# nanoporetech/vbz_compression

Measured on AMD Instinct MI355X. Metric: MB/s encode+decode, int16 signal, 1/2/4/8 MI355X vs CPU; ratio preserved, higher is better.
Workload: dtype int16

## Files before the change

### vbz_compression_amd/csrc/zstd_encode.hip

```cpp
#include "vbz_kernels.h"
#include "zstd_entropy.h"

namespace vbzhip {

namespace {

constexpr int WAVE = 64;
constexpr uint32_t BLOCK_MAX = 128u << 10;
constexpr uint32_t MIN_BLOCK = 4096;
constexpr uint32_t HUF_BLOCK_MAX = 92u << 10;
constexpr uint32_t SPLIT_MIN = 2048;
constexpr int MAXBLK = 16;
#ifndef VBZ_SPAN_BLOCK_KB
#define VBZ_SPAN_BLOCK_KB 16
#endif
constexpr uint32_t SPAN_BLOCK = VBZ_SPAN_BLOCK_KB << 10;
#ifndef VBZ_SPAN_SMALL_BLOCKS
#define VBZ_SPAN_SMALL_BLOCKS 2
#endif
constexpr uint32_t SPAN_BYTES_SMALL = SPAN_BLOCK * VBZ_SPAN_SMALL_BLOCKS, SPAN_BYTES_LARGE = SPAN_BLOCK * MAXBLK;
constexpr uint32_t SPAN_LARGE_FROM = 256u << 20;
#ifndef VBZ_KEYSPAN_KB
#define VBZ_KEYSPAN_KB 8
#endif
constexpr uint32_t KEYSPAN_BYTES = VBZ_KEYSPAN_KB << 10, KEYSPAN_LARGE_FROM = 1u << 20;
#ifndef VBZ_KEYSPAN_SHARED_KB
#define VBZ_KEYSPAN_SHARED_KB 4
#endif
constexpr uint32_t KEYSPAN_BYTES_SHARED = VBZ_KEYSPAN_SHARED_KB << 10;
__host__ __device__ constexpr uint32_t keyspan_bytes_for(uint32_t K) { return K >= KEYSPAN_LARGE_FROM ? 2u * KEYSPAN_BYTES : KEYSPAN_BYTES; }
__host__ __device__ constexpr uint32_t span_bytes_for(uint32_t N) { return N >= SPAN_LARGE_FROM ? SPAN_BYTES_LARGE : SPAN_BYTES_SMALL; }
#ifndef VBZ_STEP_LANE
#define VBZ_STEP_LANE 16
#endif
constexpr int STEP_LANE = VBZ_STEP_LANE;
static_assert(STEP_LANE == 16, "the packing step is written for 16 symbols per lane");
constexpr int STEP_DW = STEP_LANE / 4;
constexpr int STEP_SYMS = WAVE * STEP_LANE;
constexpr int OBUF_WORDS = (STEP_SYMS * 11) / 32 + 8;

struct EncSpan
{
    uint32_t read;
    uint32_t r0, r1;
    uint32_t flags;
    uint64_t tmp_off;
    uint32_t tmp_cap;
    uint32_t ord;
};
constexpr uint32_t SPAN_FIRST = 1, SPAN_LAST = 2, SPAN_KEYSEQ = 4, SPAN_SKIP = 8;
constexpr uint32_t SPAN_SHARED = 16;
constexpr uint32_t SPAN_TREE = 32;

constexpr uint32_t SHSPAN_BYTES = 8u << 10, SHSPAN_BATCH_FROM = 20u << 20;
constexpr uint32_t SHSPAN_BYTES_LARGE = 4u * SPAN_BLOCK;
constexpr uint32_t SHSPAN_MIN_REGION = 2u * SHSPAN_BYTES;

struct SpanRegion
{
    uint32_t hist[256];
    uint32_t done;
    uint32_t nshared;
    uint32_t mode;
    uint32_t treeSize, huffLog;
    uint32_t pad0[3];
    uint32_t ctable[256];
    uint32_t tree[34];
    uint32_t pad1[2];
};
constexpr uint32_t SPANREGION_ZEROED = 264;
static_assert(sizeof(SpanRegion) % 16 == 0 && offsetof(SpanRegion, ctable) == 4 * SPANREGION_ZEROED, "SpanRegion");

struct EncLds
{
    uint32_t hist[256];
    uint2 ctable[256];
    uint8_t nbBits[256];
    uint8_t weights[260];
    uint8_t tree[136];
    int32_t treeSize;
    uint32_t mode;
    uint32_t huffLog;
    uint32_t rankcnt[16];
    union
    {
        HufPmWksp pm;
        FseWeightWksp fw;
        struct
        {
            uint32_t ssize[WAVE];
            uint32_t sbeg[WAVE];
            uint32_t scnt[WAVE];
            uint32_t obuf[OBUF_WORDS];
            uint16_t seqcode[8 + 256];
            uint32_t seqpiece[256];
        };
    };
    SeqCTables seq;
    uint32_t cp[64];
    uint32_t cpCount, cpSpacing;
    __device__ __forceinline__ void set_code(uint32_t s, uint32_t code, uint32_t nb) { ctable[s] = make_uint2(code, nb); }
};

struct TableLds
{
    uint32_t hist[256];
    uint32_t ctable[256];
    uint8_t nbBits[256];
    uint8_t weights[260];
    uint8_t tree[136];
    int32_t treeSize;
    uint32_t mode;
    uint32_t huffLog;
    uint32_t rankcnt[16];
    union
    {
        HufPmWksp pm;
        FseWeightWksp fw;
    };
    __device__ __forceinline__ void set_code(uint32_t s, uint32_t code, uint32_t nb) { ctable[s] = code | (nb << 16); }
};
struct TokSeqLds
{
    uint32_t obuf[128];
    uint16_t seqcode[8 + 256];
    uint32_t seqpiece[256];
    SeqCTables seq;
    uint32_t cp[64];
    uint32_t cpCount, cpSpacing;
};

__device__ __forceinline__ void put_le(uint8_t* p, uint64_t v, int n)
{
    for (int i = 0; i < n; ++i) {
        uint32_t byte = (uint32_t)(v >> (8 * i)) & 0xFFu;
        asm volatile("" : "+v"(byte));
        p[i] = (uint8_t)byte;
    }
}

__device__ __forceinline__ uint32_t wave_sum_u32(uint32_t v)
{
    return (uint32_t)__builtin_amdgcn_readlane((int)wave_incl_scan_u32(v), 63);
}

__device__ __forceinline__ uint32_t wave_max_u32(uint32_t v)
{
#define VBZ_DPP_MAX(ctrl, rowmask) do { const uint32_t o_ = (uint32_t)__builtin_amdgcn_update_dpp(0, (int)v, ctrl, rowmask, 0xF, false); v = o_ > v ? o_ : v; } while (0)
    VBZ_DPP_MAX(0x111, 0xF);
    VBZ_DPP_MAX(0x112, 0xF);
    VBZ_DPP_MAX(0x114, 0xF);
    VBZ_DPP_MAX(0x118, 0xF);
    VBZ_DPP_MAX(0x142, 0xA);
    VBZ_DPP_MAX(0x143, 0xC);
#undef VBZ_DPP_MAX
    return (uint32_t)__builtin_amdgcn_readlane((int)v, 63);
}

constexpr uint32_t HIST_SAMPLE_FROM = 32u << 10, HIST_SAMPLE_SEEN = 240;

__device__ __forceinline__ uint32_t hist_sample_bytes(const uint8_t* in, uint32_t n)
{
    const uint32_t head = (uint32_t)((16u - ((uintptr_t)in & 15u)) & 15u);
    const uint32_t h = head < n ? head : n;
    const uint32_t nvec = (n - h) >> 4, tail0 = h + (nvec << 4);
    const uint32_t stripes = (nvec + WAVE - 1) / WAVE, groups = stripes >> 2, last = stripes & 3u;
    uint32_t chunks = groups * WAVE;
    if (last) chunks += (nvec - groups * 4u * WAVE) < (uint32_t)WAVE ? (nvec - groups * 4u * WAVE) : (uint32_t)WAVE;
    return h + (n - tail0) + 16u * chunks;
}

template <class LDS>
__device__ __forceinline__ uint32_t region_histogram(LDS& L, const uint8_t* in, uint32_t n, int lane, bool allow_sample);

template <class LDS>
__device__ __forceinline__ uint32_t region_histogram_from_plan(LDS& L, const uint8_t* in, uint32_t n, int lane, bool allow_sample, const uint32_t* sample, const uint32_t* rest)
{
    uint32_t seen = 0;
    uint32_t c[4];
#pragma unroll
    for (int j = 0; j < 4; ++j) {
        c[j] = sample[lane + 64 * j];
        seen += c[j] ? 1u : 0u;
    }
    seen = wave_sum_u32(seen);
    if (allow_sample && n >= HIST_SAMPLE_FROM && seen >= HIST_SAMPLE_SEEN) {
#pragma unroll
        for (int j = 0; j < 4; ++j) L.hist[lane + 64 * j] = c[j] ? c[j] : 1u;
        wave_lds_sync();
        return hist_sample_bytes(in, n) + (256u - seen);
    }
    if (!rest) return region_histogram(L, in, n, lane, allow_sample);
#pragma unroll
    for (int j = 0; j < 4; ++j) L.hist[lane + 64 * j] = c[j] + rest[lane + 64 * j];
    wave_lds_sync();
    return n;
}

template <class LDS>
__device__ __forceinline__ uint32_t region_histogram(LDS& L, const uint8_t* in, uint32_t n, int lane, bool allow_sample)
{
    static_assert(sizeof(HufPmWksp) >= 4 * 256 * sizeof(uint32_t), "the sub-histograms live in the table-construction workspace");
    uint32_t* sub = reinterpret_cast<uint32_t*>(&L.pm);
    for (int i = lane; i < 4 * 256; i += WAVE) sub[i] = 0;
    wave_lds_sync();
    uint32_t* mine = sub + 256 * (lane & 3);
    const uint32_t head = (uint32_t)((16u - ((uintptr_t)in & 15u)) & 15u);
    const uint32_t h = head < n ? head : n;
    if ((uint32_t)lane < h) atomicAdd(&mine[in[lane]], 1u);
    const uint32_t nvec = (n - h) >> 4;
    const uint4* vp = reinterpret_cast<const uint4*>(in + h);
    const uint32_t tail0 = h + (nvec << 4);
    if (tail0 + (uint32_t)lane < n) atomicAdd(&mine[in[tail0 + lane]], 1u);
    auto count = [&](uint32_t first_stripe, uint32_t stripe_step, uint32_t trip_stripes, int loads) {
        for (uint32_t s0 = first_stripe; s0 * WAVE < nvec; s0 += trip_stripes) {
            uint4 q[4];
#pragma unroll
            for (int u = 0; u < 4; ++u) {
                const uint32_t c = (s0 + (uint32_t)u * stripe_step) * WAVE + (uint32_t)lane;
                q[u] = (u < loads && c < nvec) ? vp[c] : make_uint4(0u, 0u, 0u, 0u);
            }
#pragma unroll
            for (int u = 0; u < 4; ++u) {
                const uint32_t c = (s0 + (uint32_t)u * stripe_step) * WAVE + (uint32_t)lane;
                if (u < loads && c < nvec) {
                    const uint32_t w[4] = { q[u].x, q[u].y, q[u].z, q[u].w };
#pragma unroll
                    for (int k = 0; k < 4; ++k) {
#pragma unroll
                        for (int j = 0; j < 4; ++j) atomicAdd(&mine[(w[k] >> (8 * j)) & 0xFFu], 1u);
                    }
                }
            }
        }
    };
    auto total = [&]() -> uint32_t {
        wave_lds_sync();
        uint32_t seen = 0;
        for (int i = lane; i < 256; i += WAVE) {
            const uint32_t c = sub[i] + sub[256 + i] + sub[512 + i] + sub[768 + i];
            L.hist[i] = c;
            seen += c ? 1u : 0u;
        }
        seen = wave_sum_u32(seen);
        wave_lds_sync();
        return seen;
    };
    if (allow_sample && n >= HIST_SAMPLE_FROM) {
        count(0, 4, 16, 4);
        const uint32_t seen = total();
        if (seen >= HIST_SAMPLE_SEEN) {
            for (int i = lane; i < 256; i += WAVE)
                if (L.hist[i] == 0) L.hist[i] = 1;
            wave_lds_sync();
            return hist_sample_bytes(in, n) + (256u - seen);
        }
        count(1, 1, 4, 3);
    } else {
        count(0, 1, 4, 4);
    }
    (void)total();
    return n;
}

#define SUB(k) do { if (tsub) { unsigned long long tn = __builtin_readcyclecounter(); tsub[k] += tn - *tl; *tl = tn; } } while (0)
template <bool STRICT>
__device__ __forceinline__ uint32_t sorted_count(const uint32_t* arr, uint32_t v, uint32_t top)
{
    uint32_t lo = 0;
    for (uint32_t step = top; step; step >>= 1) {
        const uint32_t x = arr[lo + step - 1];
        lo += (STRICT ? x < v : x <= v) ? step : 0u;
    }
    return lo;
}

template <class LDS>
__device__ __forceinline__ uint32_t huf_build_wave(LDS& L, uint32_t maxSym, uint32_t maxNbBits, int lane, unsigned long long* tsub = nullptr, unsigned long long* tl = nullptr)
{
    HufPmWksp& K = L.pm;
    uint32_t key[4];
    {
        const uint4 h = *reinterpret_cast<const uint4*>(&L.hist[4 * lane]);
        const uint32_t c[4] = { h.x, h.y, h.z, h.w };
#pragma unroll
        for (int j = 0; j < 4; ++j) {
            const uint32_t sy = 4u * (uint32_t)lane + (uint32_t)j;
            key[j] = (sy <= maxSym && c[j]) ? ((c[j] << 8) | (255u - sy)) : 0xFFFFFFFFu;
        }
    }
    for (int i = lane; i < (HUF_MAX_BITS + 1) * 16; i += WAVE) (&K.isPkg[0][0])[i] = 0;
#pragma unroll
    for (int k = 2; k <= 256; k <<= 1) {
#pragma unroll
        for (int d = k >> 1; d > 0; d >>= 1) {
            if (d >= 4) {
                const int m = d >> 2;
                const bool up = ((4 * lane) & k) == 0, lower = (lane & m) == 0;
                const bool keep_min = lower == up;
#pragma unroll
                for (int j = 0; j < 4; ++j) {
                    const uint32_t o = (uint32_t)__shfl_xor((int)key[j], m, 64);
                    const uint32_t mn = o < key[j] ? o : key[j], mx = o < key[j] ? key[j] : o;
                    key[j] = keep_min ? mn : mx;
                }
            } else {
#pragma unroll
                for (int a = 0; a < 4; ++a) {
                    const int bb = a ^ d;
                    if (bb > a) {
                        const bool up = ((4 * lane + a) & k) == 0;
                        const uint32_t mn = key[a] < key[bb] ? key[a] : key[bb], mx = key[a] < key[bb] ? key[bb] : key[a];
                        key[a] = up ? mn : mx;
                        key[bb] = up ? mx : mn;
                    }
                }
            }
        }
    }
    uint32_t n = 0;
    {
        uint32_t w4 = 0;
        uint4 lf;
        uint32_t* lfp = &lf.x;
#pragma unroll
        for (int j = 0; j < 4; ++j) {
            const bool present = key[j] != 0xFFFFFFFFu;
            n += (uint32_t)__popcll(__ballot(present));
            lfp[j] = present ? key[j] >> 8 : 0xFFFFFFFFu;
            w4 |= (255u - (key[j] & 255u)) << (8 * j);
        }
        *reinterpret_cast<uint4*>(&K.leaf[4 * lane]) = lf;
        *reinterpret_cast<uint32_t*>(&K.sym[4 * lane]) = w4;
    }
    wave_lds_sync();
    SUB(6);
    const uint32_t X0 = 2u * n - 2u;
    const uint32_t nj = (n + 63u) >> 6;
    constexpr uint32_t PM_INF = 0xFFFFFFFFu;
    uint32_t ln[4] = { 0, 0, 0, 0 };
    uint32_t lk[8];
    {
        uint4 a = make_uint4(PM_INF, PM_INF, PM_INF, PM_INF), c = a;
        if (lane < 32) {
            a = *reinterpret_cast<const uint4*>(&K.leaf[8 * lane]);
            c = *reinterpret_cast<const uint4*>(&K.leaf[8 * lane + 4]);
        }
        const uint32_t w8[8] = { a.x, a.y, a.z, a.w, c.x, c.y, c.z, c.w };
#pragma unroll
        for (int r = 0; r < 8; ++r) lk[r] = w8[r] == PM_INF ? PM_INF : w8[r] << 1;
    }
    uint32_t m = n >> 1;
    uint32_t pk4[4];
#pragma unroll
    for (int q = 0; q < 4; ++q) {
        const uint32_t t = 4u * (uint32_t)lane + (uint32_t)q;
        pk4[q] = t < m ? ((((lk[2 * q] >> 1) + (lk[2 * q + 1] >> 1)) << 1) | 1u) : PM_INF;
    }
    wave_lds_sync();
    uint64_t* const masks = reinterpret_cast<uint64_t*>(K.merged);
    uint32_t levSame = maxNbBits;
    for (uint32_t lev = 2; lev <= maxNbBits; ++lev) {
        const bool last = lev == maxNbBits;
        uint32_t it[8];
        {
            const int src = 2 * (63 - lane);
#pragma unroll
            for (int r = 0; r < 8; ++r) {
                const uint32_t p = (uint32_t)__shfl((int)pk4[(7 - r) & 3], (src + ((7 - r) >> 2)) & 63, 64);
                it[r] = lane < 32 ? lk[r] : p;
            }
        }
#pragma unroll
        for (int dl = 32; dl >= 1; dl >>= 1) {
            const bool lower = (lane & dl) == 0;
#pragma unroll
            for (int r = 0; r < 8; ++r) {
                const uint32_t o = (uint32_t)__shfl_xor((int)it[r], dl, 64);
                const uint32_t mn = o < it[r] ? o : it[r], mx = o < it[r] ? it[r] : o;
                it[r] = lower ? mn : mx;
            }
        }
#pragma unroll
        for (int d = 4; d >= 1; d >>= 1) {
#pragma unroll
            for (int r = 0; r < 8; ++r) {
                if ((r & d) == 0) {
                    const uint32_t x = it[r], y = it[r | d];
                    it[r] = x < y ? x : y;
                    it[r | d] = x < y ? y : x;
                }
            }
        }
#pragma unroll
        for (int r = 0; r < 8; ++r) {
            const uint64_t bm = __ballot((it[r] & 1u) != 0 && it[r] != PM_INF);
            if (lane == 0) masks[8 * lev + (uint32_t)r] = bm;
        }
        if (last) break;
        const uint32_t size = n + m < X0 ? n + m : X0;
        m = size >> 1;
        bool same = true;
#pragma unroll
        for (int q = 0; q < 4; ++q) {
            const uint32_t t = 4u * (uint32_t)lane + (uint32_t)q;
            const uint32_t v = t < m ? ((((it[2 * q] >> 1) + (it[2 * q + 1] >> 1)) << 1) | 1u) : PM_INF;
            same = same && v == pk4[q];
            pk4[q] = v;
        }
        if (__ballot(!same) == 0) {
            levSame = lev;
            break;
        }
    }
    wave_lds_sync();
    SUB(7);
    {
        uint32_t X = X0;
        for (uint32_t lev = maxNbBits; lev >= 2 && X; --lev) {
            const uint64_t* mk = masks + 8u * (lev < levSame ? lev : levSame);
            uint32_t pk = 0;
#pragma unroll
            for (uint32_t r = 0; r < 8; ++r) {
                const uint32_t cnt = X > r ? (X - r + 7u) >> 3 : 0u;
                const uint64_t lm = cnt >= 64u ? ~0ull : ((1ull << cnt) - 1ull);
                pk += (uint32_t)__popcll(mk[r] & lm);
            }
            const uint32_t nl = X - pk;
#pragma unroll
            for (int j = 0; j < 4; ++j) ln[j] += ((uint32_t)lane + 64u * j) < nl ? 1u : 0u;
            X = 2u * pk;
        }
#pragma unroll
        for (int j = 0; j < 4; ++j) ln[j] += ((uint32_t)lane + 64u * j) < X ? 1u : 0u;
    }
    SUB(8);
    for (int i = lane; i < 256; i += WAVE) L.nbBits[i] = 0;
    if (lane < 16) L.rankcnt[lane] = 0;
    wave_lds_sync();
    maxNbBits = (uint32_t)__builtin_amdgcn_readfirstlane((int)ln[0]);
#pragma unroll
    for (int j = 0; j < 4; ++j) {
        const uint32_t e = (uint32_t)lane + 64u * j;
        if ((uint32_t)j < nj && e < n) {
            L.nbBits[K.sym[e]] = (uint8_t)ln[j];
            atomicAdd(&L.rankcnt[ln[j]], 1u);
        }
    }
    SUB(9);
    wave_lds_sync();
    uint32_t val[HUF_ABS_MAX_BITS + 1];
    {
        uint32_t minv = 0;
#pragma unroll
        for (int n = HUF_ABS_MAX_BITS; n > 0; --n) {
            const uint32_t cnt = (uint32_t)n <= maxNbBits ? L.rankcnt[n] : 0u;
            val[n] = minv;
            minv = (uint32_t)n <= maxNbBits ? ((minv + cnt) >> 1) : 0u;
        }
        val[0] = 0;
    }
    const uint64_t below = (1ull << lane) - 1ull;
#pragma unroll
    for (int j = 0; j < 4; ++j) {
        const uint32_t s = (uint32_t)lane + 64u * j;
        const uint32_t nb = L.nbBits[s];
        uint32_t code = 0;
#pragma unroll
        for (int l = 1; l <= HUF_ABS_MAX_BITS; ++l) {
            const uint64_t m = __ballot(nb == (uint32_t)l);
            if (nb == (uint32_t)l) code = val[l] + (uint32_t)__popcll(m & below);
            val[l] += (uint32_t)__popcll(m);
        }
        L.set_code(s, code, nb);
    }
    wave_lds_sync();
    return maxNbBits;
}

template <class LDS>
__device__ __forceinline__ int huf_write_tree_wave(LDS& L, uint32_t maxSym, uint32_t huffLog, int lane)
{
    FseWeightWksp& W = L.fw;
    const uint32_t wtSize = maxSym;
    const uint32_t cnt = lane <= HUF_ABS_MAX_BITS ? W.count[lane] : 0u;
    const uint64_t nz = __ballot(cnt != 0);
    const uint32_t maxCount = wave_max_u32(cnt);
    bool fast = wtSize > 1 && nz != 0 && maxCount != wtSize && maxCount != 1;
    uint32_t tableLog = 0, maxSV = 0;
    int32_t nm = 0;
    if (fast) {
        maxSV = 63u - (uint32_t)__builtin_clzll(nz);
        tableLog = optimal_table_log(6, wtSize, maxSV, 2);
        const uint32_t total = wtSize;
        const uint64_t scale = 62 - tableLog, step = (1ull << 62) / total, vStep = 1ull << (scale - 20);
        const uint32_t lowThreshold = total >> tableLog;
        int32_t pm = 0;
        if ((uint32_t)lane <= maxSV && cnt) {
            if (cnt <= lowThreshold) nm = 1;
            else {
                int32_t proba = (int32_t)(int16_t)(((uint64_t)cnt * step) >> scale);
                if (proba < 8) {
                    uint32_t rtb = 830000u;
                    rtb = proba == 0 ? 0u : proba == 1 ? 473195u : proba == 2 ? 504333u : proba == 3 ? 520860u
                        : proba == 4 ? 550000u : proba == 5 ? 700000u : proba == 6 ? 750000u : rtb;
                    const uint64_t restToBeat = vStep * rtb;
                    proba += (((uint64_t)cnt * step) - ((uint64_t)proba << scale)) > restToBeat ? 1 : 0;
                }
                nm = proba;
                pm = proba;
            }
        }
        const int32_t still = (int32_t)(1u << tableLog) - (int32_t)wave_sum_u32((uint32_t)nm);
        const uint32_t maxP = wave_max_u32((uint32_t)pm);
        const uint64_t atMax = __ballot(pm > 0 && (uint32_t)pm == maxP);
        const int largest = atMax ? (int)__builtin_ctzll(atMax) : 0;
        const int32_t normLargest = __shfl(nm, largest, 64);
        if (-still >= (normLargest >> 1)) fast = false;
        else if (lane == largest) nm += still;
    }
    if (fast) {
        if (lane < 16) W.norm[lane] = (int16_t)nm;
        for (int i = lane; i < 52; i += WAVE) W.bitbuf[i] = 0;
        wave_lds_sync();
        if (lane == 0) W.verdict = fse_write_ncount(L.tree + 1, 133, W.norm, maxSV, tableLog);
        const uint32_t tableSize = 1u << tableLog, tableMask = tableSize - 1u;
        const uint32_t cum = wave_incl_scan_u32((uint32_t)nm) - (uint32_t)nm;
        if (lane < 16) W.cumul[lane] = cum;
        wave_lds_sync();
        const int hsz = W.verdict;
        if (hsz < 0) fast = false;
        else {
            if ((uint32_t)lane < tableSize) {
                uint32_t sy = 0;
                for (uint32_t u = 1; u <= maxSV; ++u) sy += W.cumul[u] <= (uint32_t)lane ? 1u : 0u;
                W.tableSymbol[((uint32_t)lane * ((tableSize >> 1) + (tableSize >> 3) + 3u)) & tableMask] = (uint8_t)sy;
            }
            if ((uint32_t)lane <= maxSV) {
                uint32_t dnb, dfs = 0;
                if (nm == 0) dnb = ((tableLog + 1) << 16) - tableSize;
                else if (nm == 1) { dnb = (tableLog << 16) - tableSize; dfs = cum - 1u; }
                else {
                    const uint32_t maxBitsOut = tableLog - (uint32_t)hb32((uint32_t)nm - 1u);
                    dnb = (maxBitsOut << 16) - ((uint32_t)nm << maxBitsOut);
                    dfs = cum - (uint32_t)nm;
                }
                W.deltaNbBits[lane] = dnb;
                W.deltaFindState[lane] = (int32_t)dfs;
            }
            wave_lds_sync();
            {
                const bool cell = (uint32_t)lane < tableSize;
                const uint32_t sy = cell ? W.tableSymbol[lane] : 0xFFu;
                uint32_t rank = 0;
                const uint64_t below = (1ull << lane) - 1ull;
                for (uint32_t u = 0; u <= maxSV; ++u) {
                    const uint64_t same = __ballot(sy == u);
                    if (sy == u) rank = (uint32_t)__popcll(same & below);
                }
                if (cell) W.stateTable[W.cumul[sy] + rank] = (uint16_t)(tableSize + (uint32_t)lane);
            }
            wave_lds_sync();
            const uint32_t ne = wtSize - 2u;
            if (lane < 2) {
                const uint32_t s0 = L.weights[wtSize - 1u - (uint32_t)lane];
                const uint32_t d0 = W.deltaNbBits[s0], nb0 = (d0 + (1u << 15)) >> 16;
                uint32_t st = W.stateTable[(int32_t)(((nb0 << 16) - d0) >> nb0) + W.deltaFindState[s0]];
                for (uint32_t k = (uint32_t)lane; k < ne; k += 2) {
                    const uint32_t sy = L.weights[wtSize - 3u - k];
                    const uint32_t nbo = (st + W.deltaNbBits[sy]) >> 16;
                    W.emit[k] = (uint16_t)((st & ((1u << nbo) - 1u)) | (nbo << 8));
                    st = W.stateTable[(int32_t)(st >> nbo) + W.deltaFindState[sy]];
                }
                const uint32_t slot = ne + (((wtSize & 1u) != 0) == (lane == 1) ? 0u : 1u);
                W.emit[slot] = (uint16_t)((st & tableMask) | (tableLog << 8));
                if (lane == 0) W.emit[ne + 2u] = (uint16_t)(1u | (1u << 8));
            }
            wave_lds_sync();
            uint32_t acc = 0, tb = 0;
#pragma unroll
            for (int q = 0; q < 4; ++q) {
                const uint32_t k = 4u * (uint32_t)lane + (uint32_t)q;
                const uint32_t e = k < ne + 3u ? W.emit[k] : 0u;
                acc |= (e & 0xFFu) << tb;
                tb += e >> 8;
            }
            const uint32_t incl = wave_incl_scan_u32(tb);
            const uint32_t off = incl - tb, sh = off & 31u;
            if (tb) {
                atomicOr(&W.bitbuf[off >> 5], acc << sh);
                if (sh + tb > 32u) atomicOr(&W.bitbuf[(off >> 5) + 1u], acc >> (32u - sh));
            }
            const uint32_t nbytes = ((uint32_t)__builtin_amdgcn_readlane((int)incl, 63) + 7u) >> 3;
            wave_lds_sync();
// ... 2232 lines not shown
```

Before: 609,100.

## Add one-symbol-per-lane Huffman builder fast path for alphabets up to 64 symbols

```diff
diff --git a/vbz_compression_amd/csrc/zstd_encode.hip b/vbz_compression_amd/csrc/zstd_encode.hip
--- a/vbz_compression_amd/csrc/zstd_encode.hip
+++ b/vbz_compression_amd/csrc/zstd_encode.hip
@@ -275,6 +275,151 @@
     return lo;
 }
 
+template <int M>
+__device__ __forceinline__ uint32_t lane_xor_u32(uint32_t v)
+{
+    if constexpr (M == 1) return (uint32_t)__builtin_amdgcn_mov_dpp((int)v, 0xB1, 0xF, 0xF, false);
+    else if constexpr (M == 2) return (uint32_t)__builtin_amdgcn_mov_dpp((int)v, 0x4E, 0xF, 0xF, false);
+    else if constexpr (M < 32) return (uint32_t)__builtin_amdgcn_ds_swizzle((int)v, 0x1F | (M << 10));
+    else return (uint32_t)__shfl_xor((int)v, M, 64);
+}
+
+template <class LDS>
+__device__ __forceinline__ uint32_t huf_build_wave_small(LDS& L, uint32_t maxSym, uint32_t maxNbBits, uint32_t n, const uint32_t (&c)[4], int lane,
+                                                         unsigned long long* tsub, unsigned long long* tl)
+{
+    HufPmWksp& K = L.pm;
+    constexpr uint32_t PM_INF = 0xFFFFFFFFu;
+    {
+        uint32_t np = 0;
+#pragma unroll
+        for (int j = 0; j < 4; ++j) np += (4u * (uint32_t)lane + (uint32_t)j <= maxSym && c[j]) ? 1u : 0u;
+        uint32_t pos = wave_incl_scan_u32(np) - np;
+#pragma unroll
+        for (int j = 0; j < 4; ++j) {
+            const uint32_t sy = 4u * (uint32_t)lane + (uint32_t)j;
+            if (sy <= maxSym && c[j]) K.leaf[pos++] = (c[j] << 8) | (255u - sy);
+        }
+    }
+    wave_lds_sync();
+    uint32_t key = (uint32_t)lane < n ? K.leaf[lane] : PM_INF;
+#define VBZ_SORT_STAGE(k, d) do { const uint32_t o_ = lane_xor_u32<d>(key); \
+        const bool keep_min_ = ((lane & (d)) == 0) == ((lane & (k)) == 0); \
+        key = keep_min_ ? (o_ < key ? o_ : key) : (o_ < key ? key : o_); } while (0)
+    VBZ_SORT_STAGE(2, 1);
+    VBZ_SORT_STAGE(4, 2); VBZ_SORT_STAGE(4, 1);
+    VBZ_SORT_STAGE(8, 4); VBZ_SORT_STAGE(8, 2); VBZ_SORT_STAGE(8, 1);
+    VBZ_SORT_STAGE(16, 8); VBZ_SORT_STAGE(16, 4); VBZ_SORT_STAGE(16, 2); VBZ_SORT_STAGE(16, 1);
+    VBZ_SORT_STAGE(32, 16); VBZ_SORT_STAGE(32, 8); VBZ_SORT_STAGE(32, 4); VBZ_SORT_STAGE(32, 2); VBZ_SORT_STAGE(32, 1);
+    VBZ_SORT_STAGE(64, 32); VBZ_SORT_STAGE(64, 16); VBZ_SORT_STAGE(64, 8); VBZ_SORT_STAGE(64, 4); VBZ_SORT_STAGE(64, 2); VBZ_SORT_STAGE(64, 1);
+#undef VBZ_SORT_STAGE
+    SUB(6);
+    const uint32_t X0 = 2u * n - 2u;
+    uint32_t lk[2];
+#pragma unroll
+    for (int r = 0; r < 2; ++r) {
+        const uint32_t v = (uint32_t)__shfl((int)key, (2 * lane + r) & 63, 64);
+        lk[r] = (lane < 32 && v != PM_INF) ? (v >> 8) << 1 : PM_INF;
+    }
+    uint32_t m = n >> 1;
+    uint32_t pk = (uint32_t)lane < m ? ((((lk[0] >> 1) + (lk[1] >> 1)) << 1) | 1u) : PM_INF;
+    uint64_t* const masks = reinterpret_cast<uint64_t*>(K.merged);
+    uint32_t levSame = maxNbBits;
+    for (uint32_t lev = 2; lev <= maxNbBits; ++lev) {
+        const bool last = lev == maxNbBits;
+        uint32_t it[2];
+        {
+            const int src = 2 * (63 - lane);
+#pragma unroll
+            for (int r = 0; r < 2; ++r) {
+                const uint32_t p = (uint32_t)__shfl((int)pk, (src + 1 - r) & 63, 64);
+                it[r] = lane < 32 ? lk[r] : p;
+            }
+        }
+#define VBZ_MERGE_STAGE(dl) do { const bool lower_ = (lane & (dl)) == 0; \
+        for (int r = 0; r < 2; ++r) { const uint32_t o_ = lane_xor_u32<dl>(it[r]); \
+            it[r] = lower_ ? (o_ < it[r] ? o_ : it[r]) : (o_ < it[r] ? it[r] : o_); } } while (0)
+        VBZ_MERGE_STAGE(32); VBZ_MERGE_STAGE(16); VBZ_MERGE_STAGE(8); VBZ_MERGE_STAGE(4); VBZ_MERGE_STAGE(2); VBZ_MERGE_STAGE(1);
+#undef VBZ_MERGE_STAGE
+        {
+            const uint32_t x = it[0], y = it[1];
+            it[0] = x < y ? x : y;
+            it[1] = x < y ? y : x;
+        }
+#pragma unroll
+        for (int r = 0; r < 2; ++r) {
+            const uint64_t bm = __ballot((it[r] & 1u) != 0 && it[r] != PM_INF);
+            if (lane == 0) masks[2 * lev + (uint32_t)r] = bm;
+        }
+        if (last) break;
+        const uint32_t size = n + m < X0 ? n + m : X0;
+        m = size >> 1;
+        const uint32_t v = (uint32_t)lane < m ? ((((it[0] >> 1) + (it[1] >> 1)) << 1) | 1u) : PM_INF;
+        const bool same = v == pk;
+        pk = v;
+        if (__ballot(!same) == 0) {
+            levSame = lev;
+            break;
+        }
+    }
+    wave_lds_sync();
+    SUB(7);
+    uint32_t ln = 0;
+    {
+        uint32_t X = X0;
+        for (uint32_t lev = maxNbBits; lev >= 2 && X; --lev) {
+            const uint64_t* mk = masks + 2u * (lev < levSame ? lev : levSame);
+            uint32_t npk = 0;
+#pragma unroll
+            for (uint32_t r = 0; r < 2; ++r) {
+                const uint32_t cnt = X > r ? (X - r + 1u) >> 1 : 0u;
+                npk += (uint32_t)__popcll(mk[r] & ((1ull << cnt) - 1ull));
+            }
+            ln += (uint32_t)lane < X - npk ? 1u : 0u;
+            X = 2u * npk;
+        }
+        ln += (uint32_t)lane < X ? 1u : 0u;
+    }
+    SUB(8);
+    for (int i = lane; i < 256; i += WAVE) L.nbBits[i] = 0;
+    wave_lds_sync();
+    maxNbBits = (uint32_t)__builtin_amdgcn_readfirstlane((int)ln);
+    if ((uint32_t)lane < n) L.nbBits[255u - (key & 255u)] = (uint8_t)ln;
+    uint32_t val[HUF_ABS_MAX_BITS + 1];
+    {
+        uint32_t minv = 0;
+#pragma unroll
+        for (int l = HUF_ABS_MAX_BITS; l > 0; --l) {
+            const uint32_t cnt = (uint32_t)__popcll(__ballot((uint32_t)lane < n && ln == (uint32_t)l));
+            val[l] = minv;
+            minv = (uint32_t)l <= maxNbBits ? ((minv + cnt) >> 1) : 0u;
+        }
+        val[0] = 0;
+    }
+    SUB(9);
+    wave_lds_sync();
+    const uint64_t below = (1ull << lane) - 1ull;
+#pragma unroll
+    for (int j = 0; j < 4; ++j) {
+        const uint32_t s = (uint32_t)lane + 64u * j;
+        if (64u * j > maxSym) {
+            L.set_code(s, 0u, 0u);
+            continue;
+        }
+        const uint32_t nb = L.nbBits[s];
+        uint32_t code = 0;
+#pragma unroll
+        for (int l = 1; l <= HUF_ABS_MAX_BITS; ++l) {
+            const uint64_t mm = __ballot(nb == (uint32_t)l);
+            if (nb == (uint32_t)l) code = val[l] + (uint32_t)__popcll(mm & below);
+            val[l] += (uint32_t)__popcll(mm);
+        }
+        L.set_code(s, code, nb);
+    }
+    wave_lds_sync();
+    return maxNbBits;
+}
+
 template <class LDS>
 __device__ __forceinline__ uint32_t huf_build_wave(LDS& L, uint32_t maxSym, uint32_t maxNbBits, int lane, unsigned long long* tsub = nullptr, unsigned long long* tl = nullptr)
 {
@@ -283,13 +428,20 @@
     {
         const uint4 h = *reinterpret_cast<const uint4*>(&L.hist[4 * lane]);
         const uint32_t c[4] = { h.x, h.y, h.z, h.w };
+        uint32_t np = 0;
+#pragma unroll
+        for (int j = 0; j < 4; ++j) {
+            const uint32_t sy = 4u * (uint32_t)lane + (uint32_t)j;
+            np += (uint32_t)__popcll(__ballot(sy <= maxSym && c[j]));
+        }
+        if (np <= 64u) return huf_build_wave_small(L, maxSym, maxNbBits, np, c, lane, tsub, tl);
+        for (int i = lane; i < (HUF_MAX_BITS + 1) * 16; i += WAVE) (&K.isPkg[0][0])[i] = 0;
 #pragma unroll
         for (int j = 0; j < 4; ++j) {
             const uint32_t sy = 4u * (uint32_t)lane + (uint32_t)j;
             key[j] = (sy <= maxSym && c[j]) ? ((c[j] << 8) | (255u - sy)) : 0xFFFFFFFFu;
         }
     }
-    for (int i = lane; i < (HUF_MAX_BITS + 1) * 16; i += WAVE) (&K.isPkg[0][0])[i] = 0;
 #pragma unroll
     for (int k = 2; k <= 256; k <<= 1) {
 #pragma unroll
```

Measured after the change: 613,800 (median of 6 runs). Within noise of the previous version (+0.8%).
